# vadimkantorov/convasr

Measured on AMD Instinct MI355X. Metric: audio-seconds/sec/node (fwd+bwd+CTC) at bs64x15s, higher is better.
Workload: dtype bf16

## Files before the change

### convasr_amd/csrc/conv.hip

```cpp
#include "conv_common.h"

template <typename T, bool ALIGNED> __device__ __forceinline__ uint4 load_chunk(const T* row, int e0, int n_valid) {
	constexpr int EPC = 16 / sizeof(T);
	uint4 v = make_uint4(0, 0, 0, 0);
	if (ALIGNED) {
		if (e0 + EPC <= n_valid) v = *reinterpret_cast<const uint4*>(row + e0);
		else if (e0 < n_valid) {
			T tmp[EPC];
#pragma unroll
			for (int i = 0; i < EPC; ++i) tmp[i] = (e0 + i < n_valid) ? row[e0 + i] : (T)0;
			v = *reinterpret_cast<uint4*>(tmp);
		}
	} else if (e0 < n_valid) {
		T tmp[EPC];
#pragma unroll
		for (int i = 0; i < EPC; ++i) tmp[i] = (e0 + i < n_valid) ? row[e0 + i] : (T)0;
		v = *reinterpret_cast<uint4*>(tmp);
	}
	return v;
}

template <typename T, typename O, int XI, bool ALIGNED_X, bool SK = false>
__global__ __launch_bounds__(NTHREADS, sizeof(T) == 4 ? 1 : 2) void conv1d_igemm_kernel(ConvParams p) {
	extern __shared__ __attribute__((aligned(16))) char smem[];
// ... 65 lines not shown
	constexpr bool TWO_LEVEL = sizeof(T) == 4;
	double total[2][2][16];
	if (TWO_LEVEL) {
#pragma unroll
		for (int i = 0; i < 2; ++i)
#pragma unroll
			for (int j = 0; j < 2; ++j)
#pragma unroll
				for (int k = 0; k < 16; ++k) total[i][j][k] = 0.0;
	}

	load_x(0);
	load_w(0, 0);
	store_x(0);
	store_w(0);
	__syncthreads();

	const int Q = n_cib * p.K;
	int cib = 0, tap = 0;
	const int wrow0 = wn * 64 + r, wrow1 = wrow0 + 32;
	const int woff0 = (wrow0 >> 1) << 8, wpar0 = (wrow0 & 1) << 3, wsw0 = (wrow0 >> 1) & 7;
	const int woff1 = (wrow1 >> 1) << 8, wpar1 = (wrow1 & 1) << 3, wsw1 = (wrow1 >> 1) & 7;

	for (int q = 0; q < Q; ++q) {
		const bool has_next = q + 1 < Q;
		const bool last_tap = tap == p.K - 1;
		const bool next_x = has_next && last_tap;
		if (has_next) load_w(last_tap ? cib + 1 : cib, last_tap ? 0 : tap + 1);
		if (tap == 0 && cib + 1 < n_cib) load_x(cib + 1);

		const char* xs = xbuf + (cib & 1) * xbytes;
		const char* ws = wbuf + (q & 1) * (BN * ROW_BYTES);
		const int xrow0 = (wm * 64 + r) * p.stride + tap * p.dil, xrow1 = xrow0 + 32 * p.stride;
		const int xoff0 = (xrow0 >> 1) << 8, xpar0 = (xrow0 & 1) << 3, xsw0 = (xrow0 >> 1) & 7;
		const int xoff1 = (xrow1 >> 1) << 8, xpar1 = (xrow1 & 1) << 3, xsw1 = (xrow1 >> 1) & 7;
#pragma unroll
		for (int kk = 0; kk < 4; ++kk) {
			const int chunk = kk * 2 + h;
			const uint4 a0 = *reinterpret_cast<const uint4*>(xs + xoff0 + ((xpar0 | (chunk ^ xsw0)) << 4));
			const uint4 a1 = *reinterpret_cast<const uint4*>(xs + xoff1 + ((xpar1 | (chunk ^ xsw1)) << 4));
			const uint4 b0 = *reinterpret_cast<const uint4*>(ws + woff0 + ((wpar0 | (chunk ^ wsw0)) << 4));
			const uint4 b1 = *reinterpret_cast<const uint4*>(ws + woff1 + ((wpar1 | (chunk ^ wsw1)) << 4));
			Mma<T>::run(a0, b0, acc[0][0]);
			Mma<T>::run(a0, b1, acc[0][1]);
			Mma<T>::run(a1, b0, acc[1][0]);
			Mma<T>::run(a1, b1, acc[1][1]);
		}

		if (has_next) store_w((q + 1) & 1);
		if (next_x) store_x((cib + 1) & 1);
		if (TWO_LEVEL) {
#pragma unroll
			for (int i = 0; i < 2; ++i)
#pragma unroll
				for (int j = 0; j < 2; ++j)
#pragma unroll
					for (int k = 0; k < 16; ++k) { total[i][j][k] += (double)acc[i][j][k]; acc[i][j][k] = 0.f; }
		}
		__syncthreads();
		if (last_tap) { tap = 0; ++cib; } else ++tap;
	}
	if (TWO_LEVEL) {
#pragma unroll
		for (int i = 0; i < 2; ++i)
#pragma unroll
			for (int j = 0; j < 2; ++j)
#pragma unroll
				for (int k = 0; k < 16; ++k) acc[i][j][k] = (float)total[i][j][k];
	}

	constexpr int OPITCH = BN * sizeof(O) + 16;
	char* const otile = smem;
	float* const red = reinterpret_cast<float*>(smem + BM * OPITCH);
	const int nvalid = valid_len(p.xlen, b, p.Tout);
	const ActConst ac = act_const(p.act, p.act_lo, p.act_hi);
#pragma unroll
	for (int ni = 0; ni < 2; ++ni) {
		const int col = wn * 64 + ni * 32 + r, co = co0 + col;
		const bool cok = co < p.Cout;
		const float bias = (p.bias && cok) ? p.bias[co] : 0.f;
		const float sc = (p.scale && cok) ? p.scale[co] : 1.f, sh = (p.scale && cok) ? p.shift[co] : 0.f;
		float s1 = 0.f, s2 = 0.f;
#pragma unroll
		for (int mi = 0; mi < 2; ++mi) {
#pragma unroll
			for (int g = 0; g < 16; ++g) {
				const int row = wm * 64 + mi * 32 + (g & 3) + 8 * (g >> 2) + 4 * h;
				const int t = t0 + row;
				float val = acc[mi][ni][g] + bias;
				if (t < p.Tout) { s1 += val; s2 += val * val; }
				val = apply_act(val * sc + sh, ac);
				if (t >= nvalid) val = 0.f;
				Elem<O>::store(reinterpret_cast<O*>(otile + row * OPITCH) + col, val);
			}
		}
		if (p.stats) {
			s1 += __shfl_xor(s1, 32, 64);
			s2 += __shfl_xor(s2, 32, 64);
			if (h == 0) { red[(0 * 2 + wm) * BN + col] = s1; red[(1 * 2 + wm) * BN + col] = s2; }
		}
	}
	__syncthreads();
	if (p.stats && tid < BN && co0 + tid < p.Cout) {
		double* const prow = p.stats + (int64_t)mtile * 2 * p.Cout;
		prow[co0 + tid] = (double)red[(0 * 2 + 0) * BN + tid] + (double)red[(0 * 2 + 1) * BN + tid];
		prow[p.Cout + co0 + tid] = (double)red[(1 * 2 + 0) * BN + tid] + (double)red[(1 * 2 + 1) * BN + tid];
	}
	O* const yb = reinterpret_cast<O*>(p.y) + (SK ? (int64_t)blockIdx.y * p.split_stride : 0) + (int64_t)b * p.Tout * p.Cout;
	constexpr int OEPC = 16 / sizeof(O), OCHUNKS = BN / OEPC;
	const bool vec_ok = ((p.Cout * sizeof(O)) & 15) == 0;
	for (int e = tid; e < BM * OCHUNKS; e += NTHREADS) {
		const int row = e / OCHUNKS, ch = e % OCHUNKS;
		const int t = t0 + row, co = co0 + ch * OEPC;
		if (t >= p.Tout || co >= p.Cout) continue;
		const O* src = reinterpret_cast<const O*>(otile + row * OPITCH) + ch * OEPC;
		O* dst = yb + (int64_t)t * p.Cout + co;
		if (vec_ok && co + OEPC <= p.Cout) *reinterpret_cast<uint4*>(dst) = *reinterpret_cast<const uint4*>(src);
		else
			for (int i = 0; i < OEPC && co + i < p.Cout; ++i) dst[i] = src[i];
	}
}

extern "C" int convasr_conv_cout_pad(int cout) { return (cout + BN - 1) / BN * BN; }

template <typename T>
__global__ __launch_bounds__(256) void pack_fwd_kernel(const float* __restrict__ w, T* __restrict__ fwd, int64_t pairs, int K, int64_t tap_stride) {
	extern __shared__ float tile[];
	const int64_t lin0 = (int64_t)blockIdx.x * 256;
	const int n = (int)min((int64_t)256, pairs - lin0);
	for (int j = threadIdx.x; j < n * K; j += 256) tile[j] = w[lin0 * K + j];
	__syncthreads();
	if ((int)threadIdx.x < n)
		for (int k = 0; k < K; ++k) Elem<T>::store(fwd + k * tap_stride + lin0 + threadIdx.x, tile[threadIdx.x * K + k]);
}

template <typename T>
__global__ __launch_bounds__(256) void pack_dgrad_kernel(const T* __restrict__ fwd, T* __restrict__ dgr, int Cout, int Cin, int K, int co_pad, int ci_pad) {
	__shared__ T tile[64][66];
	const int k = blockIdx.z, co0 = blockIdx.y * 64, ci0 = blockIdx.x * 64;
	const int tx = threadIdx.x & 63, ty = threadIdx.x >> 6;
	const T* src = fwd + (int64_t)k * co_pad * Cin;
	T* dst = dgr + (int64_t)(K - 1 - k) * ci_pad * Cout;
#pragma unroll 4
	for (int i = 0; i < 16; ++i) {
		const int co = co0 + ty + 4 * i, ci = ci0 + tx;
		if (co < Cout && ci < Cin) tile[ty + 4 * i][tx] = src[(int64_t)co * Cin + ci];
	}
	__syncthreads();
#pragma unroll 4
	for (int i = 0; i < 16; ++i) {
		const int ci = ci0 + ty + 4 * i, co = co0 + tx;
		if (co < Cout && ci < Cin) dst[(int64_t)ci * Cout + co] = tile[tx][ty + 4 * i];
	}
}

template <typename H> __global__ __launch_bounds__(256) void pack_fwd_half2_kernel(const float* __restrict__ w, H* __restrict__ fwd, int64_t pairs, int K, int64_t tap_stride) {
	extern __shared__ float tile[];
	const int64_t lin0 = (int64_t)blockIdx.x * 512;
	const int n = (int)min((int64_t)512, pairs - lin0);
	for (int j = threadIdx.x; j < n * K; j += 256) tile[j] = w[lin0 * K + j];
	__syncthreads();
	const int t2 = threadIdx.x * 2;
	if (t2 < n)
		for (int k = 0; k < K; ++k) {
			*reinterpret_cast<unsigned*>(fwd + k * tap_stride + lin0 + t2) = pack16<H>(tile[t2 * K + k], tile[(t2 + 1) * K + k]);
		}
}

__global__ __launch_bounds__(256) void pack_dgrad_half2_kernel(const unsigned short* __restrict__ fwd, unsigned short* __restrict__ dgr, int Cout, int Cin, int K, int co_pad, int ci_pad) {
	__shared__ unsigned short tile[64][66];
	const int k = blockIdx.z, co0 = blockIdx.y * 64, ci0 = blockIdx.x * 64;
	const int tx = threadIdx.x & 31, ty = threadIdx.x >> 5;
	const unsigned short* src = fwd + (int64_t)k * co_pad * Cin;
	unsigned short* dst = dgr + (int64_t)(K - 1 - k) * ci_pad * Cout;
#pragma unroll 4
	for (int i = 0; i < 8; ++i) {
		const int co = co0 + ty + 8 * i, ci = ci0 + 2 * tx;
		if (co < Cout && ci < Cin) {
			const unsigned v = *reinterpret_cast<const unsigned*>(src + (int64_t)co * Cin + ci);
			tile[ty + 8 * i][2 * tx] = (unsigned short)(v & 0xffffu);
			tile[ty + 8 * i][2 * tx + 1] = (unsigned short)(v >> 16);
		}
	}
	__syncthreads();
#pragma unroll 4
	for (int i = 0; i < 8; ++i) {
		const int ci = ci0 + ty + 8 * i, co = co0 + 2 * tx;
		if (co < Cout && ci < Cin)
			*reinterpret_cast<unsigned*>(dst + (int64_t)ci * Cout + co) = (unsigned)tile[2 * tx][ty + 8 * i] | ((unsigned)tile[2 * tx + 1][ty + 8 * i] << 16);
	}
}

struct PackItem { const unsigned short* src; unsigned short* dst; int Cout, Cin, K, co_pad, ci_pad, first; };
__global__ __launch_bounds__(256) void pack_dgrad_grouped_kernel(const PackItem* __restrict__ items, int n_items) {
	__shared__ unsigned short tile[64][66];
	int lo = 0, hi = n_items - 1;
	while (lo < hi) {
		const int mid = (lo + hi + 1) >> 1;
		if (items[mid].first <= (int)blockIdx.x) lo = mid; else hi = mid - 1;
	}
	const PackItem it = items[lo];
	const int local = blockIdx.x - it.first;
	const int nci = (it.Cin + 63) / 64, nco = (it.Cout + 63) / 64;
	const int ci0 = (local % nci) * 64, co0 = ((local / nci) % nco) * 64, k = local / (nci * nco);
	const int tx = threadIdx.x & 31, ty = threadIdx.x >> 5;
	const unsigned short* src = it.src + (int64_t)k * it.co_pad * it.Cin;
	unsigned short* dst = it.dst + (int64_t)(it.K - 1 - k) * it.ci_pad * it.Cout;
#pragma unroll 4
	for (int i = 0; i < 8; ++i) {
		const int co = co0 + ty + 8 * i, ci = ci0 + 2 * tx;
		if (co < it.Cout && ci < it.Cin) {
			const unsigned v = *reinterpret_cast<const unsigned*>(src + (int64_t)co * it.Cin + ci);
			tile[ty + 8 * i][2 * tx] = (unsigned short)(v & 0xffffu);
			tile[ty + 8 * i][2 * tx + 1] = (unsigned short)(v >> 16);
		}
	}
	__syncthreads();
#pragma unroll 4
	for (int i = 0; i < 8; ++i) {
		const int ci = ci0 + ty + 8 * i, co = co0 + 2 * tx;
		if (co < it.Cout && ci < it.Cin)
			*reinterpret_cast<unsigned*>(dst + (int64_t)ci * it.Cout + co) = (unsigned)tile[2 * tx][ty + 8 * i] | ((unsigned)tile[2 * tx + 1][ty + 8 * i] << 16);
	}
}

extern "C" int convasr_pack_dgrad_item_bytes(void) { return (int)sizeof(PackItem); }
extern "C" int convasr_pack_dgrad_grouped(const void* items, int n_items, int total_blocks, void* stream) {
	CONVASR_CHECK_ARG(items && n_items > 0 && total_blocks > 0, "pack_dgrad_grouped: bad arguments");
	hipLaunchKernelGGL(pack_dgrad_grouped_kernel, dim3(total_blocks), dim3(256), 0, (hipStream_t)stream, (const PackItem*)items, n_items);
	CONVASR_CHECK_LAUNCH("pack_dgrad_grouped");
	return 0;
}

template <typename T>
__global__ __launch_bounds__(256) void pack_fwd_kmajor_kernel(const float* __restrict__ w, T* __restrict__ fwd, int64_t per_tap, int64_t tap_stride, int K) {
	const int64_t n8 = per_tap >> 3;
	for (int64_t i = (int64_t)blockIdx.x * 256 + threadIdx.x; i < n8 * K; i += (int64_t)gridDim.x * 256) {
		const int64_t k = i / n8, j = (i - k * n8) << 3;
		float v[8];
		load8<float>(w + k * per_tap + j, v);
		store8<T>(fwd + k * tap_stride + j, v);
	}
}

template <typename T> static int launch_pack(const float* w, void* fwd, void* dgr, int Cout, int Cin, int K, int w_layout, hipStream_t s) {
	const int co_pad = convasr_conv_cout_pad(Cout), ci_pad = convasr_conv_cout_pad(Cin);
	const int64_t pairs = (int64_t)Cout * Cin;
	const bool x2 = sizeof(T) == 2 && (Cin & 1) == 0 && (Cout & 1) == 0 && (size_t)512 * K * sizeof(float) <= 64 * 1024;
	if (w != nullptr) {
		if (w_layout == CONVASR_W_KMAJOR) {
			if ((pairs & 7) != 0) return convasr_fail(CONVASR_EUNSUPPORTED, "pack_conv_weight: K-major source needs Cout * Cin %% 8 == 0");
			if ((const void*)w != (const void*)fwd || sizeof(T) != 4 || co_pad != Cout) {
				int64_t blocks = ceil_div64((pairs >> 3) * K, 256);
				if (blocks > 2048) blocks = 2048;
				hipLaunchKernelGGL((pack_fwd_kmajor_kernel<T>), dim3((unsigned)blocks), dim3(256), 0, s, w, (T*)fwd, pairs, (int64_t)co_pad * Cin, K);
			}
		} else if (x2) { if constexpr (sizeof(T) == 2) hipLaunchKernelGGL((pack_fwd_half2_kernel<T>), dim3((unsigned)ceil_div64(pairs, 512)), dim3(256), (size_t)512 * K * sizeof(float), s, w, (T*)fwd, pairs, K, (int64_t)co_pad * Cin); }
		else hipLaunchKernelGGL((pack_fwd_kernel<T>), dim3((unsigned)ceil_div64(pairs, 256)), dim3(256), (size_t)256 * K * sizeof(float), s, w, (T*)fwd, pairs, K, (int64_t)co_pad * Cin);
	}
	if (dgr) {
		if (x2) hipLaunchKernelGGL(pack_dgrad_half2_kernel, dim3((Cin + 63) / 64, (Cout + 63) / 64, K), dim3(256), 0, s, (const unsigned short*)fwd, (unsigned short*)dgr, Cout, Cin, K, co_pad, ci_pad);
		else hipLaunchKernelGGL((pack_dgrad_kernel<T>), dim3((Cin + 63) / 64, (Cout + 63) / 64, K), dim3(256), 0, s, (const T*)fwd, (T*)dgr, Cout, Cin, K, co_pad, ci_pad);
	}
	return 0;
}

extern "C" int convasr_pack_conv_weight(const float* w, void* packed_fwd, void* packed_dgrad, int dtype, int Cout, int Cin, int K, int w_layout, void* stream) {
	CONVASR_CHECK_ARG(packed_fwd && (w || packed_dgrad) && Cout > 0 && Cin > 0 && K > 0 && K <= 64 && (w_layout == CONVASR_W_REFERENCE || w_layout == CONVASR_W_KMAJOR), "pack_conv_weight: bad arguments (packed_fwd is required; packed_dgrad is derived from it; w NULL = packed_fwd is current)");
	int rc;
	if (dtype == CONVASR_F32) rc = launch_pack<float>(w, packed_fwd, packed_dgrad, Cout, Cin, K, w_layout, (hipStream_t)stream);
	else if (dtype == CONVASR_BF16) rc = launch_pack<bf16_t>(w, packed_fwd, packed_dgrad, Cout, Cin, K, w_layout, (hipStream_t)stream);
	else if (dtype == CONVASR_F16) rc = launch_pack<f16_t>(w, packed_fwd, packed_dgrad, Cout, Cin, K, w_layout, (hipStream_t)stream);
	else return convasr_fail(CONVASR_EUNSUPPORTED, "pack_conv_weight: dtype %d", dtype);
	if (rc) return rc;
	CONVASR_CHECK_LAUNCH("pack_conv_weight");
	return 0;
}

template <typename T, typename O, int XI, bool AL, bool SK = false> static int launch_conv(const ConvParams& p, size_t smem, hipStream_t s) {
	auto kern = conv1d_igemm_kernel<T, O, XI, AL, SK>;
	static unsigned long long attr_set = 0;
	convasr_allow_160k_lds(reinterpret_cast<const void*>(kern), attr_set);
	constexpr int BK = ROW_BYTES / sizeof(T);
	const int splits = SK ? ((p.Cin + BK - 1) / BK + p.cib_per_split - 1) / p.cib_per_split : 1;
	hipLaunchKernelGGL(kern, dim3(p.total_tiles, splits), dim3(NTHREADS), smem, s, p);
	return 0;
}

template <typename T, typename O, bool SK = false> static int dispatch_conv(const ConvParams& p, size_t smem, hipStream_t s) {
	const int xi = (p.x_rows * 8 + NTHREADS - 1) / NTHREADS;
	const bool al = ((p.Cin * sizeof(T)) & 15) == 0;
	if (!al) {
		if (xi <= 9) return launch_conv<T, O, 9, false, SK>(p, smem, s);
		return convasr_fail(CONVASR_EUNSUPPORTED, "conv1d: halo too large (x_rows %d)", p.x_rows);
	}
	if (xi <= 5) return launch_conv<T, O, 5, true, SK>(p, smem, s);
	if (xi <= 9) return launch_conv<T, O, 9, true, SK>(p, smem, s);
	if (xi <= 16) return launch_conv<T, O, 16, true, SK>(p, smem, s);
	return convasr_fail(CONVASR_EUNSUPPORTED, "conv1d: halo too large (x_rows %d)", p.x_rows);
}

int convasr_conv1d_v2_try(ConvParams p, int x_dtype, int y_dtype, hipStream_t s, int* m_tiles_out);
int convasr_conv1x1_try(ConvParams p, int x_dtype, int y_dtype, hipStream_t s, int* rows_out);
int convasr_wgrad_v2_try(WgradParams& p, int dtype, hipStream_t s);
int convasr_wgrad_v2_supports(const WgradParams& p);
static int g_conv_use_v2 = 1;
static int g_conv_debug = 0;
int convasr_conv_debug_bits() { return g_conv_debug; }
extern "C" int convasr_debug_set_conv_v2(int enable) { const int prev = g_conv_use_v2; g_conv_use_v2 = enable & 1; g_conv_debug = enable >> 8; return prev; }

static int conv1d_run(const void* x, const void* wp, void* y, int x_dtype, int y_dtype, int B, int Cin, int Cout, int Tin, int Tout, int K,
                      int stride, int dil, int pad, const float* bias, double* stats, const float* scale, const float* shift, int act,
                      float act_lo, float act_hi, const float* xlen, const ConvParams* bn_fusion, int* rows_out, void* stream) {
	CONVASR_CHECK_ARG(x && wp && y && B > 0 && Cin > 0 && Cout > 0 && Tin > 0 && Tout > 0 && K > 0 && stride > 0 && dil > 0, "conv1d_fwd: bad arguments");
	CONVASR_CHECK_ARG((scale == nullptr) == (shift == nullptr), "conv1d_fwd: scale and shift go together");
	const int64_t expect = ((int64_t)Tin + 2 * (int64_t)pad - (int64_t)dil * (K - 1) - 1) / stride + 1;
	CONVASR_CHECK_ARG(Tout <= expect, "conv1d_fwd: Tout %d inconsistent with Tin %d K %d stride %d dil %d pad %d (at most %lld)", Tout, Tin, K, stride, dil, pad, (long long)expect);
	CONVASR_CHECK_ARG(x_dtype == CONVASR_F32 || convasr_is_half(x_dtype), "conv1d_fwd: x dtype %d", x_dtype);
	if (K == 1 && stride == 1 && pad == 0 && Tin == Tout && B > 1 && !xlen && !(bn_fusion && bn_fusion->bn_xlen) && !(g_conv_debug & 512) &&
	    (int64_t)B * Tin * (Cin > Cout ? Cin : Cout) * 4 < (1ll << 31)) {
		Tin = Tout = B * Tin;
		B = 1;
	}
	ConvParams p = {};
	if (bn_fusion) p = *bn_fusion;
	p.x = x; p.w = wp; p.y = y; p.bias = bias; p.stats = stats; p.scale = scale; p.shift = shift; p.xlen = xlen;
	p.B = B; p.Cin = Cin; p.Cout = Cout; p.CoutPad = convasr_conv_cout_pad(Cout); p.Tin = Tin; p.Tout = Tout; p.K = K; p.stride = stride; p.dil = dil; p.pad = pad;
	p.act = act; p.act_lo = act_lo; p.act_hi = act_hi; p.debug = g_conv_debug;
	p.m_tiles_per_b = (Tout + BM - 1) / BM;
	p.n_tiles = p.CoutPad / BN;
	p.total_tiles = B * p.m_tiles_per_b * p.n_tiles;
	int xr = (BM - 1) * stride + (K - 1) * dil + 1;
	p.x_rows = (xr + 1) & ~1;
	const size_t osz = y_dtype == CONVASR_F32 ? 4 : 2;
	size_t smem = 2 * (size_t)p.x_rows * ROW_BYTES + 2 * BN * ROW_BYTES;
	const size_t epi = (size_t)BM * (BN * osz + 16) + 4 * BN * sizeof(float);
	if (epi > smem) smem = epi;
	CONVASR_CHECK_ARG(smem <= 160 * 1024, "conv1d_fwd: tile needs %zu B of LDS", smem);
	hipStream_t s = (hipStream_t)stream;
	int v2_rows = 0;
	if (convasr_is_half(x_dtype) && g_conv_use_v2 && convasr_conv1x1_try(p, x_dtype, y_dtype, s, &v2_rows)) {
		CONVASR_CHECK_LAUNCH("conv1d_fwd (1x1)");
		if (rows_out) *rows_out = v2_rows;
		return 0;
	}
	if (convasr_is_half(x_dtype) && g_conv_use_v2 && convasr_conv1d_v2_try(p, x_dtype, y_dtype, s, &v2_rows)) {
		CONVASR_CHECK_LAUNCH("conv1d_fwd (v2)");
		if (rows_out) *rows_out = v2_rows;
		return 0;
	}
	if (p.bn_y) return 1;
	int rc;
	if (x_dtype == CONVASR_F32 && y_dtype == CONVASR_F32) rc = dispatch_conv<float, float>(p, smem, s);
	else if (x_dtype == CONVASR_BF16 && y_dtype == CONVASR_BF16) rc = dispatch_conv<bf16_t, bf16_t>(p, smem, s);
	else if (x_dtype == CONVASR_BF16 && y_dtype == CONVASR_F32) rc = dispatch_conv<bf16_t, float>(p, smem, s);
	else if (x_dtype == CONVASR_F16 && y_dtype == CONVASR_F16) rc = dispatch_conv<f16_t, f16_t>(p, smem, s);
	else if (x_dtype == CONVASR_F16 && y_dtype == CONVASR_F32) rc = dispatch_conv<f16_t, float>(p, smem, s);
	else return convasr_fail(CONVASR_EUNSUPPORTED, "conv1d_fwd: dtype %d -> %d", x_dtype, y_dtype);
	if (rc) return rc;
	CONVASR_CHECK_LAUNCH("conv1d_fwd");
	if (rows_out) *rows_out = B * p.m_tiles_per_b;
	return 0;
}

extern "C" int convasr_conv1d_fwd(const void* x, const void* wp, void* y, int x_dtype, int y_dtype, int B, int Cin, int Cout, int Tin, int Tout, int K,
                                  int stride, int dil, int pad, const float* bias, double* stats, const float* scale, const float* shift, int act,
                                  float act_lo, float act_hi, const float* xlen, int* stats_rows, void* stream) {
	CONVASR_CHECK_ARG(!stats || stats_rows, "conv1d_fwd: stats needs stats_rows");
	return conv1d_run(x, wp, y, x_dtype, y_dtype, B, Cin, Cout, Tin, Tout, K, stride, dil, pad, bias, stats, scale, shift, act, act_lo, act_hi, xlen, nullptr, stats_rows, stream);
}

extern "C" int convasr_conv_stats_max_rows(int B, int Tout) { return B * ((Tout + BM - 1) / BM); }

static int splitk_plan(int x_dtype, int B, int Cin, int Cout, int Tout, int* cib_per_split) {
	const bool half = convasr_is_half(x_dtype);
	const int n_cu = convasr_cu_count();
	const int n_cib = half ? Cin >> 6 : (Cin + 31) / 32;
	const int tiles = B * ((Tout + (half ? 255 : BM - 1)) / (half ? 256 : BM)) * (convasr_conv_cout_pad(Cout) / BN);
	if ((half && (Cin & 63)) || n_cib < 2 || tiles * 4 > n_cu) return 1;
	int want = n_cu / tiles;
	if (want > n_cib) want = n_cib;
	if (want > 32) want = 32;
	const int cps = (n_cib + want - 1) / want;
	*cib_per_split = cps;
	return (n_cib + cps - 1) / cps;
}

template <typename O> __global__ __launch_bounds__(256) void splitk_epilogue_kernel(const float* __restrict__ part, int splits, int64_t split_stride, O* __restrict__ y, const float* __restrict__ bias,
                                                                                     const float* __restrict__ scale, const float* __restrict__ shift, int act, float lo, float hi, const float* __restrict__ xlen, int B, int T, int C) {
	const ActConst ac = act_const(act, lo, hi);
	const int c8 = C >> 3;
	const int64_t n = (int64_t)B * T * c8;
	for (int64_t i = (int64_t)blockIdx.x * 256 + threadIdx.x; i < n; i += (int64_t)gridDim.x * 256) {
		const int64_t row = i / c8;
		const int c = (int)(i - row * c8) << 3, b = (int)(row / T), t = (int)(row - (int64_t)b * T);
		float v[8], a[8];
		double acc[8];
		load8<float>(part + row * C + c, a);
#pragma unroll
		for (int k = 0; k < 8; ++k) acc[k] = (double)a[k];
		for (int s = 1; s < splits; ++s) {
			load8<float>(part + s * split_stride + row * C + c, a);
#pragma unroll
			for (int k = 0; k < 8; ++k) acc[k] += (double)a[k];
		}
#pragma unroll
		for (int k = 0; k < 8; ++k) v[k] = (float)acc[k];
		const bool live = t < valid_len(xlen, b, T);
#pragma unroll
		for (int k = 0; k < 8; ++k) {
			float val = v[k] + (bias ? bias[c + k] : 0.f);
			val = apply_act(scale ? val * scale[c + k] + shift[c + k] : val, ac);
			v[k] = live ? val : 0.f;
		}
		store8<O>(y + row * C + c, v);
	}
}

extern "C" int convasr_conv1d_fwd_splitk_plan(int x_dtype, int B, int Cin, int Cout, int Tout, int K, int64_t* workspace_bytes) {
	int cps = 0;
	if (!(convasr_is_half(x_dtype) || x_dtype == CONVASR_F32) || B <= 0 || Cin <= 0 || Cout <= 0 || Tout <= 0 || K <= 0 || (Cout & 7) || (convasr_is_half(x_dtype) && !g_conv_use_v2)) return 1;
	const int splits = splitk_plan(x_dtype, B, Cin, Cout, Tout, &cps);
	if (workspace_bytes) *workspace_bytes = splits > 1 ? (int64_t)splits * B * Tout * Cout * 4 : 0;
	return splits;
}

extern "C" int convasr_conv1d_fwd_splitk(const void* x, const void* wp, void* y, int x_dtype, int y_dtype, int B, int Cin, int Cout, int Tin, int Tout, int K, int dil, int pad,
                                         const float* bias, const float* scale, const float* shift, int act, float act_lo, float act_hi, const float* xlen, int splits, void* workspace, void* stream) {
	const bool half = convasr_is_half(x_dtype);
	CONVASR_CHECK_ARG(x && wp && y && workspace && B > 0 && Cin > 0 && Cout > 0 && Tin > 0 && Tout > 0 && K > 0 && dil > 0 && (Cout & 7) == 0 && (half ? (y_dtype == x_dtype || y_dtype == CONVASR_F32) : (x_dtype == CONVASR_F32 && y_dtype == CONVASR_F32)), "conv1d_fwd_splitk: bad arguments (16-bit or fp32 input, Cout %% 8 == 0)");
	CONVASR_CHECK_ARG((scale == nullptr) == (shift == nullptr), "conv1d_fwd_splitk: scale and shift go together");
	CONVASR_CHECK_ARG(Tout <= (int64_t)Tin + 2 * (int64_t)pad - (int64_t)dil * (K - 1), "conv1d_fwd_splitk: Tout %d inconsistent with Tin %d K %d dil %d pad %d", Tout, Tin, K, dil, pad);
	int cps = 0;
	if (splitk_plan(x_dtype, B, Cin, Cout, Tout, &cps) != splits || splits < 2) return convasr_fail(CONVASR_EINVAL, "conv1d_fwd_splitk: splits %d is not this geometry's plan", splits);
	ConvParams p = {};
	p.x = x; p.w = wp; p.y = workspace;
	p.B = B; p.Cin = Cin; p.Cout = Cout; p.CoutPad = convasr_conv_cout_pad(Cout); p.Tin = Tin; p.Tout = Tout; p.K = K; p.stride = 1; p.dil = dil; p.pad = pad;
	p.act = CONVASR_ACT_NONE; p.debug = g_conv_debug | 2048;
	p.n_tiles = p.CoutPad / BN;
	p.cib_per_split = cps; p.split_stride = (long long)B * Tout * Cout;
	hipStream_t s = (hipStream_t)stream;
	if (half) {
		if (!convasr_conv1d_v2_try(p, x_dtype, CONVASR_F32, s, nullptr)) return convasr_fail(CONVASR_EUNSUPPORTED, "conv1d_fwd_splitk: the geometry is outside the LDS-DMA kernel's envelope");
	} else {
		p.m_tiles_per_b = (Tout + BM - 1) / BM;
		p.total_tiles = B * p.m_tiles_per_b * p.n_tiles;
		p.x_rows = ((BM - 1) + (K - 1) * dil + 1 + 1) & ~1;
		size_t smem = 2 * (size_t)p.x_rows * ROW_BYTES + 2 * BN * ROW_BYTES;
		const size_t epi = (size_t)BM * (BN * 4 + 16) + 4 * BN * sizeof(float);
		if (epi > smem) smem = epi;
		if (smem > 160 * 1024) return convasr_fail(CONVASR_EUNSUPPORTED, "conv1d_fwd_splitk: tile needs %zu B of LDS", smem);
		const int rc = dispatch_conv<float, float, true>(p, smem, s);
		if (rc) return rc;
	}
	CONVASR_CHECK_LAUNCH("conv1d_fwd_splitk");
	int64_t blocks = ceil_div64((int64_t)B * Tout * (Cout >> 3), 256);
	if (blocks > 4096) blocks = 4096;
	const dim3 g((unsigned)blocks), t(256);
	const float* part = (const float*)workspace;
	if (y_dtype == CONVASR_F32) hipLaunchKernelGGL((splitk_epilogue_kernel<float>), g, t, 0, s, part, splits, p.split_stride, (float*)y, bias, scale, shift, act, act_lo, act_hi, xlen, B, Tout, Cout);
	else if (y_dtype == CONVASR_F16) hipLaunchKernelGGL((splitk_epilogue_kernel<f16_t>), g, t, 0, s, part, splits, p.split_stride, (f16_t*)y, bias, scale, shift, act, act_lo, act_hi, xlen, B, Tout, Cout);
	else hipLaunchKernelGGL((splitk_epilogue_kernel<bf16_t>), g, t, 0, s, part, splits, p.split_stride, (bf16_t*)y, bias, scale, shift, act, act_lo, act_hi, xlen, B, Tout, Cout);
	CONVASR_CHECK_LAUNCH("conv1d_fwd_splitk (epilogue)");
	return 0;
}

extern "C" int convasr_conv1d_dgrad_bn_reduce(const void* dy, const void* packed_dgrad, void* dx, int dtype, int B, int Cout, int Cin, int T_dy, int T_dx, int K, int dil, int pad,
                                              const void* bn_y, const float* bn_scale, const float* bn_shift, const float* bn_mean, const float* bn_invstd,
                                              int bn_act, float bn_act_lo, float bn_act_hi, float dropout_p, uint64_t seed, uint64_t offset, const uint64_t* step_key,
                                              const float* bn_xlen, double* bn_sums, int* bn_rows, const uint8_t* bn_gate, void* stream) {
	CONVASR_CHECK_ARG(!bn_gate || bn_act == CONVASR_ACT_RELU || bn_act == CONVASR_ACT_HARDTANH || bn_act == CONVASR_ACT_NONE, "conv1d_dgrad_bn_reduce: the one-bit gate needs an activation whose derivative is 0 or 1");
	CONVASR_CHECK_ARG(bn_y && bn_scale && bn_shift && bn_mean && bn_invstd && bn_sums && bn_rows && dropout_p >= 0.f && dropout_p < 1.f && (Cin & 7) == 0 && convasr_is_half(dtype), "conv1d_dgrad_bn_reduce: bad arguments (dtype must be CONVASR_BF16 or CONVASR_F16)");
	ConvParams f = {};
	f.bn_y = bn_y; f.bn_scale = bn_scale; f.bn_shift = bn_shift; f.bn_mean = bn_mean; f.bn_invstd = bn_invstd; f.bn_xlen = bn_xlen; f.bn_sums = bn_sums;
	f.bn_act = bn_act; f.bn_lo = bn_act_lo; f.bn_hi = bn_act_hi; f.bn_seed = convasr_mix_seed(seed); f.bn_offset = offset; f.bn_step_key = step_key; f.bn_gate = bn_gate;
	f.bn_drop_thr = (unsigned)lrintf(dropout_p * 65536.f);
	if (f.bn_drop_thr > 65535u) f.bn_drop_thr = 65535u;
	f.bn_keep_scale = 65536.f / (float)(65536u - f.bn_drop_thr);
	return conv1d_run(dy, packed_dgrad, dx, dtype, dtype, B, Cout, Cin, T_dy, T_dx, K, 1, dil, pad, nullptr, nullptr, nullptr, nullptr, CONVASR_ACT_NONE, 0.f, 0.f, nullptr, &f, bn_rows, stream);
}

template <typename T> struct WgTile;
template <> struct WgTile<bf16_t> { static constexpr int BKT = 64, PITCH = 128 * 2 + 64, CPR = 16; };
template <> struct WgTile<f16_t> : WgTile<bf16_t> {};
template <> struct WgTile<float> { static constexpr int BKT = 32, PITCH = 128 * 4 + 16, CPR = 32; };

template <typename T, int XI, bool AL_X, bool AL_Y>
__global__ __launch_bounds__(NTHREADS, 1) void conv1d_wgrad_kernel(WgradParams p) {
	extern __shared__ __attribute__((aligned(16))) char smem[];
	constexpr int EPC = 16 / sizeof(T);
	constexpr int BKT = WgTile<T>::BKT, PITCH = WgTile<T>::PITCH, CPR = WgTile<T>::CPR;
	constexpr int YI = BKT * CPR / NTHREADS;
	const int tid = threadIdx.x, lane = tid & 63, wave = tid >> 6;
	const int wm = wave >> 1, wn = wave & 1;

	const int v = xcd_remap(blockIdx.x, p.units * p.splits);
	const int unit = v % p.units, split = v / p.units;
	const int tg = unit % p.tap_groups, ci_t = (unit / p.tap_groups) % p.ci_tiles, co_t = unit / (p.tap_groups * p.ci_tiles);
	const int co0 = co_t * 128, ci0 = ci_t * 128, tap0 = tg * WG_TG;
	const int ntaps = min(WG_TG, p.K - tap0);
	const int c_begin = split * p.chunks_per_split, c_end = min(p.total_chunks, c_begin + p.chunks_per_split);

	const int ybytes = BKT * PITCH, xbytes = p.x_rows * PITCH;
	char* const ybuf = smem;
	char* const xbuf = smem + 2 * ybytes;
	const int total_x_chunks = p.x_rows * CPR;

	uint4 yreg[YI];
	uint4 xreg[XI];
	auto load_tiles = [&](int c) {
		const int b = c / p.chunks_per_b, t0 = (c % p.chunks_per_b) * BKT;
		const T* yb = reinterpret_cast<const T*>(p.dy) + (int64_t)b * p.Tout * p.Cout;
		const T* xb = reinterpret_cast<const T*>(p.x) + (int64_t)b * p.Tin * p.Cin;
		const int tin0 = t0 * p.stride - p.pad + tap0 * p.dil;
#pragma unroll
		for (int i = 0; i < YI; ++i) {
			const int e = tid + NTHREADS * i, row = e / CPR, ch = e % CPR, t = t0 + row;
			yreg[i] = make_uint4(0, 0, 0, 0);
			if (t < p.Tout) yreg[i] = load_chunk<T, AL_Y>(yb + (int64_t)t * p.Cout, co0 + ch * EPC, p.Cout);
		}
#pragma unroll
		for (int i = 0; i < XI; ++i) {
			const int e = tid + NTHREADS * i, row = e / CPR, ch = e % CPR, tin = tin0 + row;
			xreg[i] = make_uint4(0, 0, 0, 0);
			if (e < total_x_chunks && tin >= 0 && tin < p.Tin) xreg[i] = load_chunk<T, AL_X>(xb + (int64_t)tin * p.Cin, ci0 + ch * EPC, p.Cin);
		}
	};
	auto store_tiles = [&](int buf) {
#pragma unroll
		for (int i = 0; i < YI; ++i) {
			const int e = tid + NTHREADS * i;
			*reinterpret_cast<uint4*>(ybuf + buf * ybytes + (e / CPR) * PITCH + (e % CPR) * 16) = yreg[i];
		}
#pragma unroll
		for (int i = 0; i < XI; ++i) {
			const int e = tid + NTHREADS * i;
			if (e < total_x_chunks) *reinterpret_cast<uint4*>(xbuf + buf * xbytes + (e / CPR) * PITCH + (e % CPR) * 16) = xreg[i];
		}
	};

	f32x16 acc[WG_TG][2][2];
#pragma unroll
	for (int a = 0; a < WG_TG; ++a)
#pragma unroll
		for (int i = 0; i < 2; ++i)
#pragma unroll
			for (int j = 0; j < 2; ++j)
#pragma unroll
				for (int k = 0; k < 16; ++k) acc[a][i][j][k] = 0.f;

	if (c_begin < c_end) {
		load_tiles(c_begin);
		store_tiles(0);
	}
	__syncthreads();

	for (int c = c_begin; c < c_end; ++c) {
		const int buf = (c - c_begin) & 1;
		if (c + 1 < c_end) load_tiles(c + 1);
		const char* ys = ybuf + buf * ybytes;
		const char* xs = xbuf + buf * xbytes;
		if constexpr (sizeof(T) == 2) {
			const int g4 = lane >> 4, q = (lane >> 2) & 3, pc = lane & 3;
			const int kq = 8 * (g4 >> 1) + q, colb = (g4 & 1) * 16 + 4 * pc;
#pragma unroll
			for (int kk = 0; kk < BKT / 16; ++kk) {
				uint4 a[2];
#pragma unroll
				for (int mi = 0; mi < 2; ++mi) {
					const char* ap = ys + (kk * 16 + kq) * PITCH + (wm * 64 + mi * 32 + colb) * 2;
					s16x4 lo = __builtin_amdgcn_ds_read_tr16_b64_v4i16((__attribute__((address_space(3))) s16x4*)(ap));
					s16x4 hi = __builtin_amdgcn_ds_read_tr16_b64_v4i16((__attribute__((address_space(3))) s16x4*)(ap + 4 * PITCH));
					a[mi] = make_uint4(__builtin_bit_cast(uint2, lo).x, __builtin_bit_cast(uint2, lo).y, __builtin_bit_cast(uint2, hi).x, __builtin_bit_cast(uint2, hi).y);
				}
#pragma unroll
				for (int tg_i = 0; tg_i < WG_TG; ++tg_i) {
					if (tg_i < ntaps) {
						uint4 bb[2];
#pragma unroll
						for (int ni = 0; ni < 2; ++ni) {
							const char* bp = xs + ((kk * 16 + kq) * p.stride + tg_i * p.dil) * PITCH + (wn * 64 + ni * 32 + colb) * 2;
							s16x4 lo = __builtin_amdgcn_ds_read_tr16_b64_v4i16((__attribute__((address_space(3))) s16x4*)(bp));
							s16x4 hi = __builtin_amdgcn_ds_read_tr16_b64_v4i16((__attribute__((address_space(3))) s16x4*)(bp + 4 * p.stride * PITCH));
							bb[ni] = make_uint4(__builtin_bit_cast(uint2, lo).x, __builtin_bit_cast(uint2, lo).y, __builtin_bit_cast(uint2, hi).x, __builtin_bit_cast(uint2, hi).y);
						}
#pragma unroll
						for (int mi = 0; mi < 2; ++mi)
#pragma unroll
							for (int ni = 0; ni < 2; ++ni) Mma<T>::run(a[mi], bb[ni], acc[tg_i][mi][ni]);
					}
				}
			}
		} else {
			const int r = lane & 31, h = lane >> 5;
#pragma unroll 4
			for (int k2 = 0; k2 < BKT / 2; ++k2) {
				float a[2];
#pragma unroll
				for (int mi = 0; mi < 2; ++mi) a[mi] = *reinterpret_cast<const float*>(ys + (k2 * 2 + h) * PITCH + (wm * 64 + mi * 32 + r) * 4);
#pragma unroll
				for (int tg_i = 0; tg_i < WG_TG; ++tg_i) {
					if (tg_i < ntaps) {
						float bb[2];
#pragma unroll
						for (int ni = 0; ni < 2; ++ni) bb[ni] = *reinterpret_cast<const float*>(xs + ((k2 * 2 + h) * p.stride + tg_i * p.dil) * PITCH + (wn * 64 + ni * 32 + r) * 4);
#pragma unroll
						for (int mi = 0; mi < 2; ++mi)
#pragma unroll
							for (int ni = 0; ni < 2; ++ni) acc[tg_i][mi][ni] = __builtin_amdgcn_mfma_f32_32x32x2f32(a[mi], bb[ni], acc[tg_i][mi][ni], 0, 0, 0);
					}
				}
			}
		}
		if (c + 1 < c_end) store_tiles(buf ^ 1);
		__syncthreads();
	}

	const int r = lane & 31, h = lane >> 5;
#pragma unroll
	for (int tg_i = 0; tg_i < WG_TG; ++tg_i) {
		if (tg_i < ntaps) {
			float* sl = p.slab + ((int64_t)split * p.K + tap0 + tg_i) * p.Cout * p.Cin;
#pragma unroll
			for (int mi = 0; mi < 2; ++mi)
#pragma unroll
				for (int ni = 0; ni < 2; ++ni) {
					const int ci = ci0 + wn * 64 + ni * 32 + r;
#pragma unroll
					for (int g = 0; g < 16; ++g) {
						const int co = co0 + wm * 64 + mi * 32 + (g & 3) + 8 * (g >> 2) + 4 * h;
						if (co < p.Cout && ci < p.Cin) sl[(int64_t)co * p.Cin + ci] = acc[tg_i][mi][ni][g];
					}
				}
		}
	}
}

__global__ __launch_bounds__(256) void wgrad_reduce_kernel(const float* __restrict__ slab, float* __restrict__ dw, int S, int K, int Cout, int Cin, int accumulate) {
	extern __shared__ float rbuf[];
	const int co = blockIdx.y, ci0 = blockIdx.x * 64;
	const int c = threadIdx.x & 63;
	const int64_t plane = (int64_t)Cout * Cin;
	for (int k = threadIdx.x >> 6; k < K; k += 4) {
// ... 227 lines not shown
```

Baseline: 59010.

## Add specialized narrow-output 1x1 GEMM kernel for the CTC head projection

Adds a dedicated forward kernel for pointwise convolutions with small Cout (at most 64) that output fp32, as used by the final vocabulary head. The whole weight matrix is staged once in LDS per block. Each wave then streams 16-row slabs of activations through double-buffered register loads into MFMA, using a persistent grid sized to the CU count. It is meant to replace the generic tile-based 1x1 path, whose large BN tiles waste work on a narrow N dimension. The cost is one more code path, selected by a runtime shape check and an environment variable opt-out.

```diff
diff --git a/convasr_amd/csrc/conv.hip b/convasr_amd/csrc/conv.hip
--- a/convasr_amd/csrc/conv.hip
+++ b/convasr_amd/csrc/conv.hip
@@ -391,6 +391,7 @@
 
 int convasr_conv1d_v2_try(ConvParams p, int x_dtype, int y_dtype, hipStream_t s, int* m_tiles_out);
 int convasr_conv1x1_try(ConvParams p, int x_dtype, int y_dtype, hipStream_t s, int* rows_out);
+int convasr_head1_try(const ConvParams& p, int x_dtype, int y_dtype, hipStream_t s);
 int convasr_wgrad_v2_try(WgradParams& p, int dtype, hipStream_t s);
 int convasr_wgrad_v2_supports(const WgradParams& p);
 static int g_conv_use_v2 = 1;
@@ -428,6 +429,10 @@
 	CONVASR_CHECK_ARG(smem <= 160 * 1024, "conv1d_fwd: tile needs %zu B of LDS", smem);
 	hipStream_t s = (hipStream_t)stream;
 	int v2_rows = 0;
+	if (convasr_is_half(x_dtype) && g_conv_use_v2 && !stats && convasr_head1_try(p, x_dtype, y_dtype, s)) {
+		CONVASR_CHECK_LAUNCH("conv1d_fwd (head)");
+		return 0;
+	}
 	if (convasr_is_half(x_dtype) && g_conv_use_v2 && convasr_conv1x1_try(p, x_dtype, y_dtype, s, &v2_rows)) {
 		CONVASR_CHECK_LAUNCH("conv1d_fwd (1x1)");
 		if (rows_out) *rows_out = v2_rows;
diff --git a/convasr_amd/csrc/gemm1.hip b/convasr_amd/csrc/gemm1.hip
--- /dev/null
+++ b/convasr_amd/csrc/gemm1.hip
@@ -0,0 +1,120 @@
+#include "conv_common.h"
+#include <cstdlib>
+
+#define H1_MAX_WAVES 16
+#define H1_STEPS 8
+
+struct Head1Params {
+	const void* x; const void* w; float* y; const float* bias;
+	int Cin, Cout;
+	int64_t M;
+	int tiles;
+};
+
+template <typename I, int NB> __global__ __launch_bounds__(64 * H1_MAX_WAVES) void head1_fwd_kernel(Head1Params p) {
+	extern __shared__ __attribute__((aligned(16))) char smem[];
+	const int tid = threadIdx.x, lane = tid & 63;
+	const int wave = __builtin_amdgcn_readfirstlane(tid >> 6), waves = blockDim.x >> 6;
+	const int r16 = lane & 15, kb = lane >> 4;
+	const int pitch = p.Cin * 2 + 32;
+
+	{
+		const int cpr = p.Cin >> 3;
+		const I* const wp = reinterpret_cast<const I*>(p.w);
+		for (int e = tid; e < NB * 16 * cpr; e += blockDim.x) {
+			const int n = e / cpr, ch = e - n * cpr;
+			uint4 v = make_uint4(0, 0, 0, 0);
+			if (n < p.Cout) v = *reinterpret_cast<const uint4*>(wp + (int64_t)n * p.Cin + ch * 8);
+			*reinterpret_cast<uint4*>(smem + n * pitch + ch * 16) = v;
+		}
+	}
+	__syncthreads();
+
+	const int n_steps = p.Cin >> 5;
+	const char* const wl = smem + r16 * pitch + kb * 16;
+	float bias[NB];
+#pragma unroll
+	for (int nb = 0; nb < NB; ++nb) bias[nb] = (p.bias && nb * 16 + r16 < p.Cout) ? p.bias[nb * 16 + r16] : 0.f;
+
+	for (int tile = blockIdx.x; tile < p.tiles; tile += gridDim.x) {
+		const int64_t m0 = ((int64_t)tile * waves + wave) * 16;
+		if (m0 >= p.M) break;
+		const int64_t mrow = m0 + r16 < p.M ? m0 + r16 : p.M - 1;
+		const I* const xr = reinterpret_cast<const I*>(p.x) + mrow * p.Cin + kb * 8;
+
+		f32x4 acc[NB];
+#pragma unroll
+		for (int nb = 0; nb < NB; ++nb) acc[nb] = f32x4{0.f, 0.f, 0.f, 0.f};
+
+		uint4 buf0[H1_STEPS], buf1[H1_STEPS];
+		auto load = [&](uint4* buf, int s0) {
+#pragma unroll
+			for (int j = 0; j < H1_STEPS; ++j)
+				if (s0 + j < n_steps) buf[j] = *reinterpret_cast<const uint4*>(xr + (s0 + j) * 32);
+		};
+		auto mul = [&](const uint4* buf, int s0) {
+#pragma unroll
+			for (int j = 0; j < H1_STEPS; ++j)
+				if (s0 + j < n_steps) {
+#pragma unroll
+					for (int nb = 0; nb < NB; ++nb) {
+						const uint4 b = *reinterpret_cast<const uint4*>(wl + nb * 16 * pitch + (s0 + j) * 64);
+						acc[nb] = Mma16<I>::run(buf[j], b, acc[nb]);
+					}
+				}
+		};
+		load(buf0, 0);
+		for (int s0 = 0; s0 < n_steps; s0 += 2 * H1_STEPS) {
+			load(buf1, s0 + H1_STEPS);
+			mul(buf0, s0);
+			load(buf0, s0 + 2 * H1_STEPS);
+			mul(buf1, s0 + H1_STEPS);
+		}
+
+#pragma unroll
+		for (int nb = 0; nb < NB; ++nb) {
+			const int co = nb * 16 + r16;
+#pragma unroll
+			for (int g = 0; g < 4; ++g) {
+				const int64_t m = m0 + kb * 4 + g;
+				if (m < p.M && co < p.Cout) p.y[m * p.Cout + co] = acc[nb][g] + bias[nb];
+			}
+		}
+	}
+}
+
+template <typename I> static const void* head1_kernel(int nb) {
+	if (nb == 1) return (const void*)head1_fwd_kernel<I, 1>;
+	if (nb == 2) return (const void*)head1_fwd_kernel<I, 2>;
+	if (nb == 3) return (const void*)head1_fwd_kernel<I, 3>;
+	return (const void*)head1_fwd_kernel<I, 4>;
+}
+
+int convasr_head1_try(const ConvParams& c, int x_dtype, int y_dtype, hipStream_t s) {
+	if (c.K != 1 || c.stride != 1 || c.pad != 0 || c.Tin != c.Tout || (c.Cin & 63) != 0 || c.Cout > 64) return 0;
+	if (!convasr_is_half(x_dtype) || y_dtype != CONVASR_F32 || c.stats || c.scale || c.act != CONVASR_ACT_NONE || c.xlen || c.bn_y || c.cib_per_split) return 0;
+	const int nb = (c.Cout + 15) / 16;
+	const size_t smem = (size_t)nb * 16 * (c.Cin * 2 + 32);
+	if (smem > 160 * 1024) return 0;
+	const char* const off = getenv("CONVASR_NO_GEMM1");
+	if (off && off[0] == '1' && off[1] == 0) return 0;
+	Head1Params p;
+	p.x = c.x; p.w = c.w; p.y = (float*)c.y; p.bias = c.bias; p.Cin = c.Cin; p.Cout = c.Cout; p.M = (int64_t)c.B * c.Tout;
+	const int n_cu = convasr_cu_count();
+	int waves = H1_MAX_WAVES;
+	int64_t best = -1;
+	for (int w = H1_MAX_WAVES; w >= 8; w -= 4) {
+		const int64_t tiles = ceil_div64(p.M, 16 * w), cost = ceil_div64(tiles, n_cu) * w;
+		if (best < 0 || cost < best) { best = cost; waves = w; }
+	}
+	const int64_t tiles = ceil_div64(p.M, 16 * waves);
+	if (tiles >= (1ll << 31)) return 0;
+	p.tiles = (int)tiles;
+	const bool f16 = x_dtype == CONVASR_F16;
+	const void* kern = f16 ? head1_kernel<f16_t>(nb) : head1_kernel<bf16_t>(nb);
+	static unsigned long long set[2][4] = {};
+	convasr_allow_160k_lds(kern, set[f16][nb - 1]);
+	void* args[] = {&p};
+	if (hipLaunchKernel(kern, dim3(p.tiles < n_cu ? p.tiles : n_cu), dim3(64 * waves), args, smem, s) != hipSuccess) { (void)hipGetLastError(); return 0; }
+	return 1;
+}
```

Result: no change. 59050, median of 4 (+0.1%).
